# tari-project/bulletproofs-plus

Measured on AMD Instinct MI355X. Metric: 64-bit range proofs verified/sec (batch), higher is better.
Workload: dtype u32

## Files before the change

### bulletproofs-plus_amd/csrc/msm.h

```cpp
#pragma once
#include "point.h"
#include "recode.h"
#include "scalar.h"

namespace bpp {

struct PointTables {
  const niels *tab_a;
  const niels *tab_b;
  uint32_t n_a;
  const niels *tab_a_hi;
  const struct pniels *tab_b_hi;
};
struct pniels {
  fe yplusx, yminusx, xy2d, z2;
};
__device__ const uint32_t BPP_FE_TWO[10] = {2, 0, 0, 0, 0, 0, 0, 0, 0, 0};
__device__ __forceinline__ const niels *point_ptr(const PointTables &t, uint32_t idx) {
  return idx < t.n_a ? (t.tab_a + idx) : (t.tab_b + (idx - t.n_a));
}


#ifndef BPP_SORT_THREADS
#define BPP_SORT_THREADS 1024
#endif
#define BPP_SORT_THREADS_SMALL 256
#define BPP_SORT_SMALL_GROUP_TERMS 9000u
__device__ __forceinline__ int32_t msm_term_digit(const sc *__restrict__ scalars, uint32_t si, const MsmPlan &plan, uint32_t k) {
  if (!plan.split) return msm_digit_at(scalars[si].v, plan, k);
  const sc s = scalars[si & ~BPP_TERM_HI];
  uint32_t h[8];
  msm_half_words(h, s.v, (si & BPP_TERM_HI) != 0);
  return msm_digit_at(h, plan, k);
}
template <uint32_t T>
__global__ void __launch_bounds__(T) k_msm_prelude(const sc *__restrict__ scalars, const uint32_t *__restrict__ term_sidx,
                                                   const uint32_t *__restrict__ term_pidx, const uint32_t *__restrict__ group_off,
                                                   MsmPlan plan, uint32_t dig_cap, uint32_t *__restrict__ counts,
                                                   uint32_t *__restrict__ starts, uint32_t *__restrict__ sorted,
                                                   uint32_t *__restrict__ order_win, uint32_t *__restrict__ cls_hist) {
  extern __shared__ uint32_t lds[];
  const uint32_t tid = threadIdx.x, nb = plan.nb, K = plan.K;
  const uint32_t xcd = blockIdx.x & 7u, j = blockIdx.x >> 3;
  const uint32_t g = xcd + 8u * (j / K), k = j % K;
  if (g >= plan.G) return;
  uint32_t *hist = lds, *cur = lds + nb;
  int16_t *dcache = (int16_t *)(lds + 2 * nb);
  __shared__ uint32_t part[T];
  __shared__ uint32_t cls_n[256], cls_start[256], cls_cur[256];
  const uint32_t t0 = group_off[g], ng = group_off[g + 1] - t0;
  const uint32_t region = t0 * K + k * ng;
  for (uint32_t q = tid; q < nb; q += T) hist[q] = 0;
  if (tid < 256) cls_n[tid] = cls_cur[tid] = 0;
  __syncthreads();
  for (uint32_t i0 = tid; i0 < ng; i0 += 8 * T) {
    uint32_t si[8];
    int32_t d[8];
#pragma unroll
    for (int u = 0; u < 8; u++) si[u] = (i0 + u * T < ng) ? term_sidx[t0 + i0 + u * T] : 0xffffffffu;
#pragma unroll
    for (int u = 0; u < 8; u++) d[u] = si[u] != 0xffffffffu ? msm_term_digit(scalars, si[u], plan, k) : 0;
#pragma unroll
    for (int u = 0; u < 8; u++) {
      const uint32_t i = i0 + u * T;
      if (i < ng) {
        if (i < dig_cap) dcache[i] = (int16_t)d[u];
        if (d[u]) atomicAdd(&hist[(uint32_t)(d[u] < 0 ? -d[u] : d[u]) - 1], 1u);
      }
    }
  }
  __syncthreads();
  const uint32_t per = (nb + T - 1u) / T;
  const uint32_t a = tid * per < nb ? tid * per : nb, b = (a + per < nb) ? a + per : nb;
  uint32_t sum = 0;
  for (uint32_t q = a; q < b; q++) sum += hist[q];
  part[tid] = sum;
  __syncthreads();
  for (uint32_t off = 1; off < T; off <<= 1) {
    uint32_t v = (tid >= off) ? part[tid - off] : 0;
    __syncthreads();
    part[tid] += v;
    __syncthreads();
  }
  uint32_t run = (tid == 0) ? 0 : part[tid - 1];
  const size_t bbase = ((size_t)g * K + k) * nb;
  for (uint32_t q = a; q < b; q++) {
    const uint32_t cnt = hist[q];
    counts[bbase + q] = cnt;
    starts[bbase + q] = region + run;
    cur[q] = run;
    run += cnt;
    atomicAdd(&cls_n[cnt < 255u ? cnt : 255u], 1u);
  }
  __syncthreads();
  for (uint32_t i0 = tid; i0 < ng; i0 += 8 * T) {
    int32_t d[8];
    uint32_t pi[8];
#pragma unroll
    for (int u = 0; u < 8; u++) {
      const uint32_t i = i0 + u * T;
      const bool in = i < ng;
      pi[u] = in ? term_pidx[t0 + i] : 0u;
      d[u] = !in ? 0 : (i < dig_cap ? (int32_t)dcache[i] : msm_term_digit(scalars, term_sidx[t0 + i], plan, k));
    }
#pragma unroll
    for (int u = 0; u < 8; u++)
      if (d[u]) {
        const uint32_t pos = atomicAdd(&cur[(uint32_t)(d[u] < 0 ? -d[u] : d[u]) - 1], 1u);
        sorted[region + pos] = pi[u] | (d[u] < 0 ? 0x80000000u : 0u);
      }
  }
  uint32_t *gh = cls_hist + (size_t)g * K * 768;
  if (tid < 256) part[tid] = cls_n[tid];
  __syncthreads();
  for (uint32_t off = 1; off < 256; off <<= 1) {
    uint32_t v = (tid < 256 && tid + off < 256) ? part[tid + off] : 0;
    __syncthreads();
    if (tid < 256) part[tid] += v;
    __syncthreads();
  }
  if (tid < 256) {
    cls_start[tid] = part[tid] - cls_n[tid];
    gh[k * 768 + tid] = cls_n[tid];
    gh[k * 768 + 256 + tid] = cls_start[tid];
  }
  __syncthreads();
  for (uint32_t q = a; q < b; q++) {
    const uint32_t cnt = hist[q], cls = cnt < 255u ? cnt : 255u;
    const uint32_t pos = cls_start[cls] + atomicAdd(&cls_cur[cls], 1u);
    order_win[bbase + pos] = (uint32_t)(bbase + q);
  }
}

template <uint32_t T>
__global__ void __launch_bounds__(T) k_msm_order(const uint32_t *__restrict__ counts, const uint32_t *__restrict__ order_win,
                                                 uint32_t *cls_hist, MsmPlan plan, uint32_t *__restrict__ order) {
  const uint32_t tid = threadIdx.x, g = blockIdx.x, nb = plan.nb, K = plan.K;
  __shared__ uint32_t part[256];
  uint32_t *gh = cls_hist + (size_t)g * K * 768;
  const size_t gbase = (size_t)g * K * nb;
  uint32_t tot = 0;
  if (tid < 256) {
    for (uint32_t kk = 0; kk < K; kk++) tot += gh[kk * 768 + tid];
    part[tid] = tot;
  }
  __syncthreads();
  for (uint32_t off = 1; off < 256; off <<= 1) {
    uint32_t v = (tid < 256 && tid + off < 256) ? part[tid + off] : 0;
    __syncthreads();
    if (tid < 256) part[tid] += v;
    __syncthreads();
  }
  if (tid < 256) {
    uint32_t running = part[tid] - tot;
    for (uint32_t kk = 0; kk < K; kk++) {
      gh[kk * 768 + 512 + tid] = running - gh[kk * 768 + 256 + tid];
      running += gh[kk * 768 + tid];
    }
  }
  __syncthreads();
  const uint32_t n_all = K * nb;
  for (uint32_t i0 = tid; i0 < n_all; i0 += 4 * T) {
    uint32_t bk[4], cn[4];
#pragma unroll
    for (int u = 0; u < 4; u++) bk[u] = i0 + u * T < n_all ? order_win[gbase + i0 + u * T] : 0xffffffffu;
#pragma unroll
    for (int u = 0; u < 4; u++) cn[u] = bk[u] != 0xffffffffu ? counts[bk[u]] : 0u;
#pragma unroll
    for (int u = 0; u < 4; u++)
      if (bk[u] != 0xffffffffu) {
        const uint32_t i = i0 + u * T, kk = i >> (plan.c - 1u), q = i & (nb - 1u);
        order[gbase + (uint32_t)(q + gh[kk * 768 + 512 + (cn[u] < 255u ? cn[u] : 255u)])] = bk[u];
      }
  }
}
inline uint32_t msm_prelude_dig_cap(const MsmPlan &plan, uint32_t max_group_terms, uint32_t threads = BPP_SORT_THREADS) {
  const uint32_t fixed = 2u * plan.nb * 4u + (threads + 3u * 256u) * 4u;
  const uint32_t room = fixed + 1024u < 65536u ? (65536u - 1024u - fixed) / 2u : 0u;
  return max_group_terms < room ? max_group_terms : room;
}
inline size_t msm_prelude_lds(const MsmPlan &plan, uint32_t dig_cap) { return (size_t)2 * plan.nb * 4 + (size_t)((dig_cap + 1u) & ~1u) * 2; }

__device__ __forceinline__ void msm_slice_range(uint32_t ng, uint32_t S, uint32_t s, uint32_t &lo, uint32_t &hi) {
  const uint32_t L = (ng + S - 1u) / S;
  lo = s * L < ng ? s * L : ng;
  hi = ng - lo > L ? lo + L : ng;
}
__global__ void __launch_bounds__(BPP_SLICE_THREADS) k_msm_slice_hist(const sc *__restrict__ scalars, const uint32_t *__restrict__ term_sidx,
                                                                       const uint32_t *__restrict__ group_off, MsmPlan plan, uint32_t S,
                                                                       uint32_t *__restrict__ slice_hist) {
  extern __shared__ uint32_t lds[];
  constexpr uint32_t T = BPP_SLICE_THREADS;
  const uint32_t tid = threadIdx.x, nb = plan.nb, K = plan.K;
  const uint32_t s = blockIdx.x % S, gk = blockIdx.x / S, g = gk / K, k = gk % K;
  if (g >= plan.G) return;
  const uint32_t t0 = group_off[g], ng = group_off[g + 1] - t0;
  uint32_t lo, hi;
  msm_slice_range(ng, S, s, lo, hi);
  for (uint32_t q = tid; q < nb; q += T) lds[q] = 0;
  __syncthreads();
  for (uint32_t i0 = lo + tid; i0 < hi; i0 += 4 * T) {
    uint32_t si[4];
    int32_t d[4];
#pragma unroll
    for (int u = 0; u < 4; u++) si[u] = (i0 + u * T < hi) ? term_sidx[t0 + i0 + u * T] : 0xffffffffu;
#pragma unroll
    for (int u = 0; u < 4; u++) d[u] = si[u] != 0xffffffffu ? msm_term_digit(scalars, si[u], plan, k) : 0;
#pragma unroll
    for (int u = 0; u < 4; u++)
      if (d[u]) atomicAdd(&lds[(uint32_t)(d[u] < 0 ? -d[u] : d[u]) - 1], 1u);
  }
  __syncthreads();
  uint32_t *out = slice_hist + (size_t)blockIdx.x * nb;
  for (uint32_t q = tid; q < nb; q += T) out[q] = lds[q];
}

__global__ void __launch_bounds__(BPP_SLICE_SCAN_THREADS) k_msm_slice_scan(uint32_t *__restrict__ slice_hist, const uint32_t *__restrict__ group_off,
                                                                            MsmPlan plan, uint32_t S, uint32_t *counts,
                                                                            uint32_t *__restrict__ starts, uint32_t *__restrict__ order_win,
                                                                            uint32_t *__restrict__ cls_hist) {
  constexpr uint32_t T = BPP_SLICE_SCAN_THREADS;
  const uint32_t tid = threadIdx.x, nb = plan.nb, K = plan.K;
  const uint32_t gk = blockIdx.x, g = gk / K, k = gk % K;
  if (g >= plan.G) return;
  __shared__ uint32_t part[T];
  __shared__ uint32_t cls_n[256], cls_start[256], cls_cur[256];
  const uint32_t t0 = group_off[g], ng = group_off[g + 1] - t0;
  const uint32_t region = t0 * K + k * ng;
  uint32_t *rows = slice_hist + (size_t)gk * S * nb;
  const size_t bbase = (size_t)gk * nb;
  if (tid < 256) cls_n[tid] = cls_cur[tid] = 0;
  const uint32_t per = (nb + T - 1u) / T;
  const uint32_t a = tid * per < nb ? tid * per : nb, b = (a + per < nb) ? a + per : nb;
  uint32_t sum = 0;
  for (uint32_t q = a; q < b; q++) {
    uint32_t tot = 0;
    for (uint32_t s = 0; s < S; s++) tot += rows[(size_t)s * nb + q];
    counts[bbase + q] = tot;
    sum += tot;
  }
  part[tid] = sum;
  __syncthreads();
  for (uint32_t off = 1; off < T; off <<= 1) {
    uint32_t v = (tid >= off) ? part[tid - off] : 0;
    __syncthreads();
    part[tid] += v;
    __syncthreads();
  }
  uint32_t run = (tid == 0) ? 0 : part[tid - 1];
  for (uint32_t q = a; q < b; q++) {
    const uint32_t cnt = counts[bbase + q];
    starts[bbase + q] = region + run;
    uint32_t at = run;
    for (uint32_t s = 0; s < S; s++) {
      const uint32_t h = rows[(size_t)s * nb + q];
      rows[(size_t)s * nb + q] = at;
      at += h;
    }
    run += cnt;
    atomicAdd(&cls_n[cnt < 255u ? cnt : 255u], 1u);
  }
  __syncthreads();
  uint32_t *gh = cls_hist + (size_t)g * K * 768;
  if (tid < 256) part[tid] = cls_n[tid];
  __syncthreads();
  for (uint32_t off = 1; off < 256; off <<= 1) {
    uint32_t v = (tid < 256 && tid + off < 256) ? part[tid + off] : 0;
    __syncthreads();
    if (tid < 256) part[tid] += v;
    __syncthreads();
  }
  if (tid < 256) {
    cls_start[tid] = part[tid] - cls_n[tid];
    gh[k * 768 + tid] = cls_n[tid];
    gh[k * 768 + 256 + tid] = cls_start[tid];
  }
  __syncthreads();
  for (uint32_t q = a; q < b; q++) {
    const uint32_t cnt = counts[bbase + q], cls = cnt < 255u ? cnt : 255u;
    const uint32_t pos = cls_start[cls] + atomicAdd(&cls_cur[cls], 1u);
    order_win[bbase + pos] = (uint32_t)(bbase + q);
  }
}

__global__ void __launch_bounds__(BPP_SLICE_THREADS) k_msm_slice_scatter(const sc *__restrict__ scalars, const uint32_t *__restrict__ term_sidx,
                                                                          const uint32_t *__restrict__ term_pidx,
                                                                          const uint32_t *__restrict__ group_off, MsmPlan plan, uint32_t S,
                                                                          const uint32_t *__restrict__ slice_offs, uint32_t *__restrict__ sorted) {
  extern __shared__ uint32_t lds[];
  constexpr uint32_t T = BPP_SLICE_THREADS;
  const uint32_t tid = threadIdx.x, nb = plan.nb, K = plan.K;
  const uint32_t s = blockIdx.x % S, gk = blockIdx.x / S, g = gk / K, k = gk % K;
  if (g >= plan.G) return;
  const uint32_t t0 = group_off[g], ng = group_off[g + 1] - t0;
  const uint32_t region = t0 * K + k * ng;
  uint32_t lo, hi;
  msm_slice_range(ng, S, s, lo, hi);
  if (lo >= hi) return;
  const uint32_t *offs = slice_offs + (size_t)blockIdx.x * nb;
  for (uint32_t q = tid; q < nb; q += T) lds[q] = offs[q];
  __syncthreads();
  for (uint32_t i0 = lo + tid; i0 < hi; i0 += 4 * T) {
    uint32_t si[4], pi[4];
    int32_t d[4];
#pragma unroll
    for (int u = 0; u < 4; u++) {
      const bool in = i0 + u * T < hi;
      si[u] = in ? term_sidx[t0 + i0 + u * T] : 0xffffffffu;
      pi[u] = in ? term_pidx[t0 + i0 + u * T] : 0u;
    }
#pragma unroll
    for (int u = 0; u < 4; u++) d[u] = si[u] != 0xffffffffu ? msm_term_digit(scalars, si[u], plan, k) : 0;
#pragma unroll
    for (int u = 0; u < 4; u++)
      if (d[u]) {
        const uint32_t pos = atomicAdd(&lds[(uint32_t)(d[u] < 0 ? -d[u] : d[u]) - 1], 1u);
        if (pos < ng) sorted[region + pos] = pi[u] | (d[u] < 0 ? 0x80000000u : 0u);
      }
  }
}

#ifndef BPP_ACC_WAVES
#define BPP_ACC_WAVES 3
#endif
__global__ void __launch_bounds__(64, BPP_ACC_WAVES) k_msm_accumulate(const uint32_t *__restrict__ sorted,
                                                       const uint32_t *__restrict__ starts,
                                                       const uint32_t *__restrict__ counts,
                                                       const uint32_t *__restrict__ order, PointTables tabs,
                                                       uint32_t per_group, uint32_t G, ge *__restrict__ buckets) {
  const uint32_t xcd = blockIdx.x & 7u, j = blockIdx.x >> 3;
  const uint32_t bpg = (per_group + 63u) / 64u;
  const uint32_t g = xcd + 8u * (j / bpg);
  const uint32_t slot = (j % bpg) * 64u + threadIdx.x;
  if (g >= G || slot >= per_group) return;
  const uint32_t bkt = order[(size_t)g * per_group + slot];
  const uint32_t a = starts[bkt], n = counts[bkt];
  if (n == 0) return;
  uint32_t e = sorted[a];
  niels q;
  niels_load_swapped(q, point_ptr(tabs, e & 0x7fffffffu), (e >> 31) != 0);
  ge acc;
  ge_from_niels_first(acc, q);
  fe_fence(acc.X);
  fe_fence(acc.Y);
  fe_fence(acc.T);
  if (n > 1) {
    e = sorted[a + 1];
    niels_load_swapped(q, point_ptr(tabs, e & 0x7fffffffu), (e >> 31) != 0);
  }
  uint32_t i = 1;
  while (i < n) {
    uint32_t e2 = e;
    niels q2;
    if (i + 1 < n) {
      e2 = sorted[a + i + 1];
      niels_load_swapped(q2, point_ptr(tabs, e2 & 0x7fffffffu), (e2 >> 31) != 0);
    }
    ge_madd_swapped(acc, acc, q, (e >> 31) != 0);
    if (++i >= n) break;
    if (i + 1 < n) {
      e = sorted[a + i + 1];
      niels_load_swapped(q, point_ptr(tabs, e & 0x7fffffffu), (e >> 31) != 0);
    }
    ge_madd_swapped(acc, acc, q2, (e2 >> 31) != 0);
    ++i;
  }
  buckets[bkt] = acc;
}

__global__ void __launch_bounds__(64) k_msm_window_rc(const ge *__restrict__ buckets, const uint32_t *__restrict__ counts,
                                                      MsmPlan plan, ge *__restrict__ W) {
  const uint32_t gk = blockIdx.x, lane = threadIdx.x;
  const uint32_t nb = plan.nb, lb = plan.c - 1;
  const uint32_t lBc = lb / 2, Bc = 1u << lBc, A = nb >> lBc;
  const size_t base = (size_t)gk * nb;
  __shared__ ge red[64];
  ge acc;
  ge_identity(acc);
  const bool is_row = lane < 32;
  const uint32_t idx = is_row ? lane : lane - 32;
  if (is_row ? (idx < A) : (idx < Bc)) {
    const uint32_t cnt = is_row ? Bc : A;
    for (uint32_t q = 0; q < cnt; q++) {
      const uint32_t j0 = is_row ? (Bc * idx + q) : (Bc * q + idx);
      if (counts[base + j0]) {
        const ge x = buckets[base + j0];
        ge_add(acc, acc, x);
      }
    }
  }
  red[lane] = acc;
  __syncthreads();
  const uint32_t half_n = is_row ? A : Bc;
  for (uint32_t off = 1; off < 32; off <<= 1) {
    ge y2;
    const bool act = idx + off < half_n;
    if (act) y2 = red[lane + off];
    __syncthreads();
    if (act) {
      ge_add(acc, acc, y2);
      red[lane] = acc;
    }
    __syncthreads();
  }
  if (is_row ? (idx == 0 || idx >= A) : (idx >= Bc)) ge_identity(acc);
  red[lane] = acc;
  __syncthreads();
  for (uint32_t off = 16; off >= 1; off >>= 1) {
    if (idx < off) {
      ge x = red[lane], y2 = red[lane + off];
      ge_add(x, x, y2);
      red[lane] = x;
    }
    __syncthreads();
  }
  if (lane == 0) {
    ge rows = red[0];
    const ge cols = red[32];
    if (lBc) ge_dbl_n(rows, rows, (int)lBc);
    ge_add(rows, rows, cols);
    W[gk] = rows;
  }
}

__global__ void __launch_bounds__(64) k_msm_window_rc2(const ge *__restrict__ buckets, const uint32_t *__restrict__ counts, MsmPlan plan,
                                                       uint32_t n_windows, ge *__restrict__ W) {
  const uint32_t lane = threadIdx.x;
  const uint32_t nb = plan.nb, lb = plan.c - 1;
  const uint32_t lBc = lb / 2, Bc = 1u << lBc, A = nb >> lBc;
  const bool is_row = lane < 32;
  const uint32_t sub = (lane >> 4) & 1u, idx = lane & 15u;
  const uint32_t gk = blockIdx.x * 2u + sub;
  const bool live = gk < n_windows;
  const size_t base = (size_t)gk * nb;
  __shared__ ge red[64];
  ge acc;
  ge_identity(acc);
  if (live && (is_row ? (idx < A) : (idx < Bc))) {
    const uint32_t cnt = is_row ? Bc : A;
    for (uint32_t q = 0; q < cnt; q++) {
      const uint32_t j0 = is_row ? (Bc * idx + q) : (Bc * q + idx);
      if (counts[base + j0]) {
        const ge x = buckets[base + j0];
        ge_add(acc, acc, x);
      }
    }
  }
  red[lane] = acc;
  __syncthreads();
  const uint32_t half_n = is_row ? A : Bc;
  for (uint32_t off = 1; off < 16; off <<= 1) {
    ge y2;
    const bool act = idx + off < half_n;
    if (act) y2 = red[lane + off];
    __syncthreads();
    if (act) {
      ge_add(acc, acc, y2);
      red[lane] = acc;
    }
    __syncthreads();
  }
  if (is_row ? (idx == 0 || idx >= A) : (idx >= Bc)) ge_identity(acc);
  red[lane] = acc;
  __syncthreads();
  for (uint32_t off = 8; off >= 1; off >>= 1) {
    if (idx < off) {
      ge x = red[lane], y2 = red[lane + off];
      ge_add(x, x, y2);
      red[lane] = x;
    }
    __syncthreads();
  }
  if (is_row && idx == 0 && live) {
    ge rows = red[lane];
    const ge cols = red[lane + 32];
    if (lBc) ge_dbl_n(rows, rows, (int)lBc);
    ge_add(rows, rows, cols);
    W[gk] = rows;
  }
}

__global__ void __launch_bounds__(64) k_msm_bitsum(const ge *__restrict__ buckets, const uint32_t *__restrict__ counts,
                                                   MsmPlan plan, ge *__restrict__ Q ) {
  const uint32_t b = blockIdx.x, k = blockIdx.y, g = blockIdx.z, lane = threadIdx.x;
  const uint32_t nb = plan.nb;
  const size_t base = ((size_t)g * plan.K + k) * nb;
  __shared__ ge red[64];
  ge acc;
  ge_identity(acc);
  for (uint32_t j = lane; j < nb; j += 64) {
    if ((((j + 1) >> b) & 1u) && counts[base + j] != 0) {
      const ge q = buckets[base + j];
      ge_add(acc, acc, q);
    }
  }
  red[lane] = acc;
  __syncthreads();
  for (uint32_t off = 32; off >= 1; off >>= 1) {
    if (lane < off) {
      ge x = red[lane], y2 = red[lane + off];
      ge_add(x, x, y2);
      red[lane] = x;
    }
    __syncthreads();
  }
  if (lane == 0) Q[((size_t)g * plan.K + k) * plan.c + b] = red[0];
}

__global__ void __launch_bounds__(64) k_msm_window(const ge *__restrict__ Q, MsmPlan plan, ge *__restrict__ W) {
  const uint32_t i = blockIdx.x * blockDim.x + threadIdx.x;
  if (i >= plan.G * plan.K) return;
  const ge *q = Q + (size_t)i * plan.c;
  ge acc = q[plan.c - 1];
  for (int b = (int)plan.c - 2; b >= 0; b--) {
    ge_dbl(acc, acc);
    const ge x = q[b];
    ge_add(acc, acc, x);
  }
  W[i] = acc;
}

__global__ void __launch_bounds__(64) k_msm_final(const ge *__restrict__ W, MsmPlan plan, ge *__restrict__ R,
                                                  uint32_t *__restrict__ is_identity) {
  const uint32_t g = blockIdx.x * blockDim.x + threadIdx.x;
  if (g >= plan.G) return;
  const ge *w = W + (size_t)g * plan.K;
  ge acc = w[plan.K - 1];
  for (int k = (int)plan.K - 2; k >= 0; k--) {
    ge_dbl_n(acc, acc, (uint32_t)k < plan.K_wide ? (int)plan.c : (int)plan.c - 1);
    const ge x = w[k];
    ge_add(acc, acc, x);
  }
  R[g] = acc;
  is_identity[g] = ge_is_ristretto_identity(acc) ? 1u : 0u;
}

template <int S>
__device__ __forceinline__ void quad_bcast(fe &r, const fe &v) {
  static_assert(S >= 0 && S < 4, "quad position");
#define BPP_QB(i) "v_mov_b32_dpp %" #i ", %1" #i " quad_perm:[%20,%20,%20,%20] row_mask:0xf bank_mask:0xf\n\t"
  asm volatile(BPP_QB(0) BPP_QB(1) BPP_QB(2) BPP_QB(3) BPP_QB(4) BPP_QB(5) BPP_QB(6) BPP_QB(7) BPP_QB(8) BPP_QB(9) "s_nop 0"
               : "=&v"(r.v[0]), "=&v"(r.v[1]), "=&v"(r.v[2]), "=&v"(r.v[3]), "=&v"(r.v[4]), "=&v"(r.v[5]), "=&v"(r.v[6]), "=&v"(r.v[7]),
                 "=&v"(r.v[8]), "=&v"(r.v[9])
               : "v"(v.v[0]), "v"(v.v[1]), "v"(v.v[2]), "v"(v.v[3]), "v"(v.v[4]), "v"(v.v[5]), "v"(v.v[6]), "v"(v.v[7]), "v"(v.v[8]),
                 "v"(v.v[9]), "n"(S));
#undef BPP_QB
}
struct QuadMask {
  uint64_t b1, b2, b3;
};
__device__ __forceinline__ QuadMask quad_mask(uint32_t q) {
  (void)q;
  QuadMask k;
  k.b1 = 0x2222222222222222ull;
  k.b2 = 0x4444444444444444ull;
  k.b3 = 0x8888888888888888ull;
  asm volatile("" : "+s"(k.b1), "+s"(k.b2), "+s"(k.b3));
  return k;
}
__device__ __forceinline__ void fe_sel4(fe &r, const QuadMask &k, const fe &a0, const fe &a1, const fe &a2, const fe &a3) {
#pragma unroll
  for (int i = 0; i < 10; i++) {
    uint32_t t;
    asm("v_cndmask_b32 %0, %1, %2, %5\n\tv_cndmask_b32 %0, %0, %3, %6\n\tv_cndmask_b32 %0, %0, %4, %7"
        : "=&v"(t)
        : "v"(a0.v[i]), "v"(a1.v[i]), "v"(a2.v[i]), "v"(a3.v[i]), "s"(k.b1), "s"(k.b2), "s"(k.b3));
    r.v[i] = t;
  }
}
__device__ __forceinline__ void fe_sel_lane3(fe &r, const QuadMask &k, const fe &a, const fe &b) {
#pragma unroll
  for (int i = 0; i < 10; i++) {
    uint32_t t;
    asm("v_cndmask_b32 %0, %1, %2, %3" : "=v"(t) : "v"(a.v[i]), "v"(b.v[i]), "s"(k.b3));
    r.v[i] = t;
  }
}
__device__ __forceinline__ void quad_efgh(fe &m, const QuadMask &q, const fe &E, const fe &F, const fe &G, const fe &H) {
  fe l, r;
  fe_sel4(l, q, E, G, F, E);
  fe_sel4(r, q, F, H, G, H);
  fe_mul(m, l, r);
}

__device__ __forceinline__ void quad_ge_add(fe &m, const QuadMask &q, const ge &other, const fe &d2, const fe &one) {
  fe X, Y, Z, T;
  quad_bcast<0>(X, m);
  quad_bcast<1>(Y, m);
  quad_bcast<2>(Z, m);
  quad_bcast<3>(T, m);
  fe l0, r0, l1, r1, l, r, s2;
  fe_sub(l0, Y, X);
  fe_sub(r0, other.Y, other.X);
  fe_add(l1, Y, X);
  fe_add(r1, other.Y, other.X);
  fe_sel4(l, q, l0, l1, T, Z);
  fe_sel4(r, q, r0, r1, other.T, other.Z);
  fe_mul(s2, l, r);
  fe_sel4(r, q, one, one, d2, one);
  fe_mul(s2, s2, r);
  fe a, b, c, d, e, f, gg, h;
  quad_bcast<0>(a, s2);
  quad_bcast<1>(b, s2);
  quad_bcast<2>(c, s2);
  quad_bcast<3>(d, s2);
  fe_add(d, d, d);
  fe_sub(e, b, a);
  fe_sub(f, d, c);
  fe_add(gg, d, c);
  fe_add(h, b, a);
  fe_carry(gg);
  quad_efgh(m, q, e, f, gg, h);
}
__device__ __forceinline__ void quad_ge_madd(fe &m, const QuadMask &q, const niels &pt, const fe &zz) {
  fe X, Y, Z, T;
  quad_bcast<0>(X, m);
  quad_bcast<1>(Y, m);
  quad_bcast<2>(Z, m);
  quad_bcast<3>(T, m);
  fe l0, l1, l, r, s2;
  fe_add(l0, Y, X);
  fe_sub(l1, Y, X);
  fe_sel4(l, q, l0, l1, T, Z);
  fe_sel4(r, q, pt.yplusx, pt.yminusx, pt.xy2d, zz);
  fe_mul(s2, l, r);
  fe a, b, c, d, e, f, gg, h;
  quad_bcast<0>(a, s2);
  quad_bcast<1>(b, s2);
  quad_bcast<2>(c, s2);
  quad_bcast<3>(d, s2);
  fe_sub(e, a, b);
  fe_add(h, a, b);
  fe_add(gg, d, c);
  fe_sub(f, d, c);
  fe_carry(gg);
  quad_efgh(m, q, e, f, gg, h);
}
__device__ __forceinline__ void quad_ge_dbl(fe &m, const QuadMask &q) {
  fe x, y, v, s2;
  quad_bcast<0>(x, m);
  quad_bcast<1>(y, m);
  fe_add(v, x, y);
  fe_sel_lane3(v, q, m, v);
  fe_sq(s2, v);
  fe a, b, c, t, e, f, gg, h;
  quad_bcast<0>(a, s2);
  quad_bcast<1>(b, s2);
  quad_bcast<2>(c, s2);
  quad_bcast<3>(t, s2);
  fe_add(h, a, b);
  fe_sub_lazy(e, h, t);
  fe_sub_lazy(gg, a, b);
  fe_dbl_add(f, c, gg);
  fe_carry(f);
  quad_efgh(m, q, e, f, gg, h);
}
__device__ __forceinline__ void quad_load(fe &m, const QuadMask &q, const ge &p) { fe_sel4(m, q, p.X, p.Y, p.Z, p.T); }
__device__ __forceinline__ void quad_gather(ge &p, const fe &m) {
  quad_bcast<0>(p.X, m);
  quad_bcast<1>(p.Y, m);
  quad_bcast<2>(p.Z, m);
  quad_bcast<3>(p.T, m);
}

__global__ void __launch_bounds__(64) k_msm_final_quad(const ge *__restrict__ W, MsmPlan plan, ge *__restrict__ R,
                                                       uint32_t *__restrict__ is_identity) {
  const uint32_t lane = threadIdx.x, qi = lane & 3u;
  const QuadMask q = quad_mask(qi);
  const uint32_t g = blockIdx.x * 16u + (lane >> 2);
  const bool active = g < plan.G;
  const ge *w = W + (size_t)(active ? g : plan.G - 1) * plan.K;
  fe m;
  {
    const ge top = w[plan.K - 1];
    fe_sel4(m, q, top.X, top.Y, top.Z, top.T);
  }
  fe d2, one;
  fe_const(d2, FE_D2);
  fe_1(one);
  for (int k = (int)plan.K - 2; k >= 0; k--) {
    const int n = (uint32_t)k < plan.K_wide ? (int)plan.c : (int)plan.c - 1;
#pragma unroll 1
    for (int i = 0; i < n; i++) quad_ge_dbl(m, q);
    {
      const ge wk = w[k];
      quad_ge_add(m, q, wk, d2, one);
    }
  }
  ge acc;
  quad_bcast<0>(acc.X, m);
  quad_bcast<1>(acc.Y, m);
  quad_bcast<2>(acc.Z, m);
  quad_bcast<3>(acc.T, m);
  if (active && qi == 0) {
    R[g] = acc;
    is_identity[g] = ge_is_ristretto_identity(acc) ? 1u : 0u;
  }
}

__global__ void __launch_bounds__(64) k_msm_accumulate_quad(const uint32_t *__restrict__ sorted, const uint32_t *__restrict__ starts,
                                                            const uint32_t *__restrict__ counts, const uint32_t *__restrict__ order,
                                                            PointTables tabs, uint32_t n_buckets, ge *__restrict__ buckets) {
  const uint32_t lane = threadIdx.x, qi = lane & 3u;
  const QuadMask q = quad_mask(qi);
  const uint32_t slot = blockIdx.x * 16u + (lane >> 2);
  if (slot >= n_buckets) return;
  const uint32_t bkt = order[slot];
  const uint32_t a = starts[bkt], n = counts[bkt];
  if (n == 0) return;
  fe m;
  {
    ge id;
    ge_identity(id);
    quad_load(m, q, id);
  }
  auto fetch = [&](uint32_t ent, niels &dn, fe &dz) {
    const uint32_t pi = ent & 0x3fffffffu;
    const bool hi = (ent & BPP_POINT_HI) != 0, proj = hi && pi >= tabs.n_a;
    const pniels *pp = tabs.tab_b_hi + (proj ? pi - tabs.n_a : 0u);
    const niels *np = hi ? (pi < tabs.n_a ? tabs.tab_a_hi + pi : (const niels *)pp) : point_ptr(tabs, pi);
    const fe *zp = proj ? &pp->z2 : (const fe *)BPP_FE_TWO;
    dn.yplusx = np->yplusx;
    dn.yminusx = np->yminusx;
    dn.xy2d = np->xy2d;
    dz = *zp;
  };
  uint32_t ew[4];
#pragma unroll
  for (int u = 0; u < 4; u++) ew[u] = (uint32_t)u < n ? sorted[a + u] : 0u;
  for (uint32_t i0 = 0; i0 < n; i0 += 4) {
    uint32_t ec[4];
    niels pt[4];
    fe pzz[4];
#pragma unroll
    for (int u = 0; u < 4; u++) {
      ec[u] = ew[u];
      if (i0 + u < n) fetch(ec[u], pt[u], pzz[u]);
    }
#pragma unroll
    for (int u = 0; u < 4; u++) ew[u] = i0 + 4 + u < n ? sorted[a + i0 + 4 + u] : 0u;
#pragma unroll
    for (int u = 0; u < 4; u++) {
      if (i0 + u < n) {
        niels_cneg(pt[u], (ec[u] >> 31) != 0);
        quad_ge_madd(m, q, pt[u], pzz[u]);
      }
    }
  }
  fe *dst = (fe *)(buckets + bkt);
  dst[qi] = m;
}

__global__ void __launch_bounds__(64) k_split_shift_quad(const niels *__restrict__ pts, uint32_t n, pniels *__restrict__ out) {
  const uint32_t lane = threadIdx.x, qi = lane & 3u;
  const QuadMask q = quad_mask(qi);
  const uint32_t i = blockIdx.x * 16u + (lane >> 2);
  if (i >= n) return;
  const niels p = pts[i];
  ge g;
  fe_sub(g.X, p.yplusx, p.yminusx);
  fe_carry(g.X);
  fe_add(g.Y, p.yplusx, p.yminusx);
  fe_carry(g.Y);
  fe_1(g.Z);
  g.Z.v[0] = 2;
  fe_0(g.T);
  fe m;
  quad_load(m, q, g);
#pragma unroll 1
  for (uint32_t k = 0; k < BPP_MSM_SPLIT_BIT; k++) quad_ge_dbl(m, q);
  fe X, Y, Z, T, s0, s1, md, m2, d2, o;
  quad_bcast<0>(X, m);
  quad_bcast<1>(Y, m);
  quad_bcast<2>(Z, m);
  quad_bcast<3>(T, m);
  fe_add(s0, Y, X);
  fe_sub(s1, Y, X);
  fe_const(d2, FE_D2);
  fe_mul(md, T, d2);
  fe_add(m2, Z, Z);
  fe_sel4(o, q, s0, s1, md, m2);
  fe_carry(o);
  fe *dst = (fe *)(out + i);
  dst[qi] = o;
}
__global__ void __launch_bounds__(64) k_split_shift_table(const niels *__restrict__ tab, uint32_t n, niels *__restrict__ out) {
  const uint32_t i = blockIdx.x * blockDim.x + threadIdx.x;
  if (i >= n) return;
  ge g;
  ge_identity(g);
  const niels p = tab[i];
  ge_madd(g, g, p);
  ge_dbl_n(g, g, (int)BPP_MSM_SPLIT_BIT);
  fe zi, x, y;
  fe_invert(zi, g.Z);
  fe_mul(x, g.X, zi);
  fe_mul(y, g.Y, zi);
  niels e;
  niels_from_affine(e, x, y);
  fe_carry(e.yminusx);
  out[i] = e;
}

#define BPP_RC_QUAD_SEGS 4u
__global__ void __launch_bounds__(1024) k_msm_window_rc_quad(const ge *__restrict__ buckets, const uint32_t *__restrict__ counts,
                                                             MsmPlan plan, ge *__restrict__ W) {
  const uint32_t gk = blockIdx.x, tid = threadIdx.x, qi = tid & 3u, quad = tid >> 2, lane = quad & 63u, seg = quad >> 6;
  const QuadMask q = quad_mask(qi);
  const uint32_t nb = plan.nb, lb = plan.c - 1;
  const uint32_t lBc = lb / 2, Bc = 1u << lBc, A = nb >> lBc;
  const size_t base = (size_t)gk * nb;
  __shared__ ge red[64 * BPP_RC_QUAD_SEGS];
  fe d2, one, m;
  fe_const(d2, FE_D2);
  fe_1(one);
  ge id;
  ge_identity(id);
  quad_load(m, q, id);
  const bool is_row = lane < 32;
  const uint32_t idx = is_row ? lane : lane - 32;
  if (is_row ? (idx < A) : (idx < Bc)) {
    const uint32_t cnt = is_row ? Bc : A;
    const uint32_t per = (cnt + BPP_RC_QUAD_SEGS - 1u) / BPP_RC_QUAD_SEGS;
    const uint32_t k0 = seg * per < cnt ? seg * per : cnt, k1 = k0 + per < cnt ? k0 + per : cnt;
    for (uint32_t k = k0; k < k1; k++) {
      const uint32_t j0 = is_row ? (Bc * idx + k) : (Bc * k + idx);
      if (counts[base + j0]) {
        const ge x = buckets[base + j0];
        quad_ge_add(m, q, x, d2, one);
      }
    }
  }
  fe *slot = (fe *)&red[quad];
  slot[qi] = m;
  __syncthreads();
  for (uint32_t step = 1; step < BPP_RC_QUAD_SEGS; step <<= 1) {
    const bool act = (seg % (2u * step)) == 0 && seg + step < BPP_RC_QUAD_SEGS;
    if (act) {
      const ge y2 = red[quad + 64u * step];
      quad_ge_add(m, q, y2, d2, one);
    }
    __syncthreads();
    if (act) slot[qi] = m;
    __syncthreads();
  }
  const bool lead = seg == 0;
  const uint32_t half_n = is_row ? A : Bc;
  for (uint32_t off = 1; off < 32; off <<= 1) {
    ge y2;
    const bool act = lead && idx + off < half_n;
    if (act) y2 = red[lane + off];
    __syncthreads();
    if (act) {
      quad_ge_add(m, q, y2, d2, one);
      slot[qi] = m;
    }
    __syncthreads();
  }
  if (is_row ? (idx == 0 || idx >= A) : (idx >= Bc)) quad_load(m, q, id);
  if (lead) slot[qi] = m;
  __syncthreads();
  for (uint32_t off = 16; off >= 1; off >>= 1) {
    if (lead && idx < off) {
      const ge y2 = red[lane + off];
      quad_ge_add(m, q, y2, d2, one);
      slot[qi] = m;
    }
    __syncthreads();
  }
  if (quad == 0) {
    for (uint32_t i = 0; i < lBc; i++) quad_ge_dbl(m, q);
    const ge cols = red[32];
    quad_ge_add(m, q, cols, d2, one);
    ge w;
    quad_gather(w, m);
    if (qi == 0) W[gk] = w;
  }
}

__global__ void __launch_bounds__(64) k_compress_ge(const ge *__restrict__ in, uint32_t count, uint8_t *__restrict__ out32) {
  const uint32_t i = blockIdx.x * blockDim.x + threadIdx.x;
  if (i >= count) return;
  uint8_t c32[32];
  ristretto_compress(c32, in[i]);
  uint32_t *o = (uint32_t *)(out32 + (size_t)i * 32);
#pragma unroll
  for (int k = 0; k < 8; k++)
    o[k] = (uint32_t)c32[4 * k] | ((uint32_t)c32[4 * k + 1] << 8) | ((uint32_t)c32[4 * k + 2] << 16) | ((uint32_t)c32[4 * k + 3] << 24);
}

__global__ void k_ge_to_bytes(const ge *__restrict__ R, uint32_t n, uint8_t *__restrict__ out128) {
  uint32_t i = blockIdx.x * blockDim.x + threadIdx.x;
  if (i >= n) return;
  const ge p = R[i];
  uint8_t b[32];
  fe_tobytes(b, p.X);
  for (int k = 0; k < 32; k++) out128[(size_t)i * 128 + k] = b[k];
  fe_tobytes(b, p.Y);
  for (int k = 0; k < 32; k++) out128[(size_t)i * 128 + 32 + k] = b[k];
  fe_tobytes(b, p.Z);
  for (int k = 0; k < 32; k++) out128[(size_t)i * 128 + 64 + k] = b[k];
  fe_tobytes(b, p.T);
  for (int k = 0; k < 32; k++) out128[(size_t)i * 128 + 96 + k] = b[k];
}

__global__ void __launch_bounds__(64) k_sum_accumulators(const uint8_t *__restrict__ in128, uint32_t n, uint8_t *__restrict__ comp32,
                                   uint32_t *__restrict__ is_identity) {
  if (blockIdx.x != 0 || threadIdx.x != 0) return;
  ge acc;
  ge_identity(acc);
  for (uint32_t i = 0; i < n; i++) {
    ge p;
    uint8_t b[32];
    for (int k = 0; k < 32; k++) b[k] = in128[(size_t)i * 128 + k];
    fe_frombytes(p.X, b);
    for (int k = 0; k < 32; k++) b[k] = in128[(size_t)i * 128 + 32 + k];
    fe_frombytes(p.Y, b);
    for (int k = 0; k < 32; k++) b[k] = in128[(size_t)i * 128 + 64 + k];
    fe_frombytes(p.Z, b);
    for (int k = 0; k < 32; k++) b[k] = in128[(size_t)i * 128 + 96 + k];
    fe_frombytes(p.T, b);
    ge_add(acc, acc, p);
  }
  uint8_t c32[32];
  ristretto_compress(c32, acc);
  for (int i = 0; i < 32; i++) comp32[i] = c32[i];
  is_identity[0] = ge_is_ristretto_identity(acc) ? 1u : 0u;
}

__global__ void k_shader_clock(uint64_t *out, uint32_t naps) {
  const uint64_t c0 = __builtin_amdgcn_s_memtime(), w0 = __builtin_amdgcn_s_memrealtime();
  for (uint32_t i = 0; i < naps; i++) __builtin_amdgcn_s_sleep(127);
  if (threadIdx.x == 0) {
    out[0] = __builtin_amdgcn_s_memtime() - c0;
    out[1] = __builtin_amdgcn_s_memrealtime() - w0;
  }
}

}
```

Before: 28.56 million.

## Software-pipeline bucket accumulation loads with inline asm and explicit vmcnt waits

Rewrites the bucket accumulation loop so the next sorted index and the next table entry are issued as raw global loads in inline assembly. The loop then waits on them with explicit s_waitcnt vmcnt counts, double-buffered across two register entries. Indices are clamped to the last list element so loads are always issued without branches. The intent is to overlap memory latency with the field arithmetic of the mixed addition. In exchange it relies on fragile hand-counted vmcnt values and compiler-visible ordering, and it issues redundant loads at the tail.

```diff
diff --git a/bulletproofs-plus_amd/csrc/msm.h b/bulletproofs-plus_amd/csrc/msm.h
--- a/bulletproofs-plus_amd/csrc/msm.h
+++ b/bulletproofs-plus_amd/csrc/msm.h
@@ -323,6 +323,53 @@
 #ifndef BPP_ACC_WAVES
 #define BPP_ACC_WAVES 3
 #endif
+__device__ __forceinline__ uint32_t msm_list_pos(uint32_t pos, uint32_t last) { return pos < last ? pos : last; }
+
+typedef uint32_t acc_u32x4 __attribute__((ext_vector_type(4)));
+typedef uint32_t acc_u32x2 __attribute__((ext_vector_type(2)));
+struct acc_entry {
+  acc_u32x4 a0, a1, b0, b1, c0, c1;
+  acc_u32x2 a2, b2, c2;
+};
+__device__ __forceinline__ void acc_issue_word(uint32_t &w, const uint32_t *p) {
+  asm volatile("global_load_dword %0, %1, off" : "=v"(w) : "v"(p));
+}
+__device__ __forceinline__ void acc_issue_entry(acc_entry &r, const niels *src, bool neg) {
+  const fe *pair = &src->yplusx, *pa = pair + (neg ? 1 : 0), *pb = pair + (neg ? 0 : 1);
+  asm volatile(
+      "global_load_dwordx4 %0, %9, off\n\t"
+      "global_load_dwordx4 %1, %9, off offset:16\n\t"
+      "global_load_dwordx2 %2, %9, off offset:32\n\t"
+      "global_load_dwordx4 %3, %10, off\n\t"
+      "global_load_dwordx4 %4, %10, off offset:16\n\t"
+      "global_load_dwordx2 %5, %10, off offset:32\n\t"
+      "global_load_dwordx4 %6, %11, off offset:80\n\t"
+      "global_load_dwordx4 %7, %11, off offset:96\n\t"
+      "global_load_dwordx2 %8, %11, off offset:112"
+      : "=&v"(r.a0), "=&v"(r.a1), "=&v"(r.a2), "=&v"(r.b0), "=&v"(r.b1), "=&v"(r.b2), "=&v"(r.c0), "=&v"(r.c1), "=&v"(r.c2)
+      : "v"(pa), "v"(pb), "v"(src));
+}
+static_assert(sizeof(fe) == 40 && offsetof(niels, yplusx) == 0 && offsetof(niels, yminusx) == 40 && offsetof(niels, xy2d) == 80,
+              "acc_issue_entry addresses the fields of a table line by these offsets");
+#define BPP_ACC_ENTRY_OPERANDS(r) "+v"(r.a0), "+v"(r.a1), "+v"(r.a2), "+v"(r.b0), "+v"(r.b1), "+v"(r.b2), "+v"(r.c0), "+v"(r.c1), "+v"(r.c2)
+__device__ __forceinline__ void acc_wait_word(uint32_t &w) { asm volatile("s_waitcnt vmcnt(9)" : "+v"(w)); }
+__device__ __forceinline__ void acc_wait_entry(acc_entry &r) { asm volatile("s_waitcnt vmcnt(10)" : BPP_ACC_ENTRY_OPERANDS(r)); }
+__device__ __forceinline__ void acc_drain(uint32_t &keep, ge *&out) {
+  __builtin_amdgcn_sched_barrier(0);
+  asm volatile("s_waitcnt vmcnt(0)" : "+v"(keep), "+s"(out));
+  __builtin_amdgcn_sched_barrier(0);
+}
+__device__ __forceinline__ void acc_entry_niels(niels &q, const acc_entry &r) {
+#pragma unroll
+  for (int k = 0; k < 4; k++) {
+    q.yplusx.v[k] = r.a0[k], q.yplusx.v[4 + k] = r.a1[k];
+    q.yminusx.v[k] = r.b0[k], q.yminusx.v[4 + k] = r.b1[k];
+    q.xy2d.v[k] = r.c0[k], q.xy2d.v[4 + k] = r.c1[k];
+  }
+#pragma unroll
+  for (int k = 0; k < 2; k++) q.yplusx.v[8 + k] = r.a2[k], q.yminusx.v[8 + k] = r.b2[k], q.xy2d.v[8 + k] = r.c2[k];
+}
+
 __global__ void __launch_bounds__(64, BPP_ACC_WAVES) k_msm_accumulate(const uint32_t *__restrict__ sorted,
                                                        const uint32_t *__restrict__ starts,
                                                        const uint32_t *__restrict__ counts,
@@ -336,36 +383,48 @@
   const uint32_t bkt = order[(size_t)g * per_group + slot];
   const uint32_t a = starts[bkt], n = counts[bkt];
   if (n == 0) return;
-  uint32_t e = sorted[a];
+  const uint32_t *list = sorted + a;
+  const uint32_t last = n - 1u;
+  const uint32_t e0 = list[0], e1 = list[msm_list_pos(1u, last)];
   niels q;
-  niels_load_swapped(q, point_ptr(tabs, e & 0x7fffffffu), (e >> 31) != 0);
+  niels_load_swapped(q, point_ptr(tabs, e0 & 0x7fffffffu), (e0 >> 31) != 0);
   ge acc;
   ge_from_niels_first(acc, q);
   fe_fence(acc.X);
   fe_fence(acc.Y);
   fe_fence(acc.T);
-  if (n > 1) {
-    e = sorted[a + 1];
-    niels_load_swapped(q, point_ptr(tabs, e & 0x7fffffffu), (e >> 31) != 0);
-  }
+  uint32_t wx, wy;
+  acc_entry ra, rb;
+  bool neg_a = (e1 >> 31) != 0, neg_b;
+  acc_issue_word(wx, list + msm_list_pos(2u, last));
+  acc_issue_entry(ra, point_ptr(tabs, e1 & 0x7fffffffu), neg_a);
   uint32_t i = 1;
   while (i < n) {
-    uint32_t e2 = e;
-    niels q2;
-    if (i + 1 < n) {
-      e2 = sorted[a + i + 1];
-      niels_load_swapped(q2, point_ptr(tabs, e2 & 0x7fffffffu), (e2 >> 31) != 0);
-    }
-    ge_madd_swapped(acc, acc, q, (e >> 31) != 0);
+    acc_wait_word(wx);
+    neg_b = (wx >> 31) != 0;
+    acc_issue_word(wy, list + msm_list_pos(i + 2u, last));
+    acc_issue_entry(rb, point_ptr(tabs, wx & 0x7fffffffu), neg_b);
+    acc_wait_entry(ra);
+    acc_entry_niels(q, ra);
+    ge_madd_swapped(acc, acc, q, neg_a);
     if (++i >= n) break;
-    if (i + 1 < n) {
-      e = sorted[a + i + 1];
-      niels_load_swapped(q, point_ptr(tabs, e & 0x7fffffffu), (e >> 31) != 0);
-    }
-    ge_madd_swapped(acc, acc, q2, (e2 >> 31) != 0);
+    acc_wait_word(wy);
+    neg_a = (wy >> 31) != 0;
+    acc_issue_word(wx, list + msm_list_pos(i + 2u, last));
+    acc_issue_entry(ra, point_ptr(tabs, wy & 0x7fffffffu), neg_a);
+    acc_wait_entry(rb);
+    acc_entry_niels(q, rb);
+    ge_madd_swapped(acc, acc, q, neg_b);
     ++i;
   }
-  buckets[bkt] = acc;
+  uint32_t out = bkt;
+  ge *dst = buckets;
+  acc_drain(out, dst);
+  fe_fence(acc.X);
+  fe_fence(acc.Y);
+  fe_fence(acc.Z);
+  fe_fence(acc.T);
+  dst[out] = acc;
 }
 
 __global__ void __launch_bounds__(64) k_msm_window_rc(const ge *__restrict__ buckets, const uint32_t *__restrict__ counts,
```

After: 28.47 million, median of 2. About the same (-0.3%).
